# cunningham-lab/cyclic-gps

Hardware: AMD Instinct MI355X
Metric: block-tridiag solve+log-det (mahal_and_det) algorithmic GB/s vs HBM roofline, N=2^20 d=4 on one GPU, N=2^24 d=4 time-axis sharded on several; solves/s alongside (higher is better)
Workload: dtype f64; 1 GPU; BASELINE config 2: mahal_and_det on ONE SPD block-tridiagonal system, N=1048576 block rows (1048576 per GPU), d=4, conditioned bidiagonal-factor generator seed 1234; rows_total=1048576, rows_per_gpu=1048576, d=4, algorithmic_bytes=301989776, parallelism=single GPU, algo=tile-fused

## Files before the change

__graft_entry__.py:

```python
import os
import subprocess
import sys

ROOT = os.path.dirname(os.path.abspath(__file__))
PKG = os.path.join(ROOT, "cyclic-gps_amd")
CSRC = os.path.join(PKG, "csrc")
LIB = os.path.join(PKG, "lib", "libcgps.so")
HIPCC = os.environ.get("HIPCC", "/opt/rocm/bin/hipcc")


def _stale(target, sources):
    if not os.path.exists(target):
        return True
    t = os.path.getmtime(target)
    return any(os.path.getmtime(s) > t for s in sources)


UNITS = ("cgps_core", "cgps_mahal", "cgps_decompose", "cgps_solve", "cgps_inverse", "cgps_leg", "cgps_sample",
         "cgps_leg_obs")
FLAGS = ["--offload-arch=gfx950", "-O3", "-std=c++17", "-fPIC", "-Wno-unused-value"]
FLAGS += os.environ.get("CGPS_CXXFLAGS", "").split()


def _compile_unit(args):
    src, obj = args
    cmd = [HIPCC] + FLAGS + ["-c", src, "-o", obj]
    print("[build]", " ".join(cmd), flush=True)
    subprocess.check_call(cmd, cwd=ROOT)
    return obj


def build_oracle():
    if ROOT not in sys.path:
        sys.path.insert(0, ROOT)
    from oracle import cr_oracle


def build(force=False):
    from concurrent.futures import ThreadPoolExecutor
    hdrs = [os.path.join(CSRC, f) for f in sorted(os.listdir(CSRC)) if f.endswith(".h")]
    hdrs.append(os.path.join(ROOT, "include", "cgps.h"))
    objdir = os.path.join(PKG, "lib", "obj")
    os.makedirs(objdir, exist_ok=True)
    jobs, objs = [], []
    stamp = os.path.join(objdir, ".flags")
    flag_key = " ".join(FLAGS)
    flags_changed = (open(stamp).read() if os.path.exists(stamp) else None) != flag_key
    for u in UNITS:
        src, obj = os.path.join(CSRC, u + ".hip"), os.path.join(objdir, u + ".o")
        objs.append(obj)
        if force or flags_changed or _stale(obj, [src] + hdrs):
            jobs.append((src, obj))
    if jobs:
        with ThreadPoolExecutor(max_workers=min(len(jobs), os.cpu_count() or 4)) as ex:
            list(ex.map(_compile_unit, jobs))
        with open(stamp, "w") as fh:
            fh.write(flag_key)
    if jobs or _stale(LIB, objs):
        cmd = [HIPCC, "--offload-arch=gfx950", "-shared", "-fPIC", "-o", LIB] + objs
        print("[build]", " ".join(cmd), flush=True)
        subprocess.check_call(cmd, cwd=ROOT)
    for p in (ROOT, PKG):
        if p not in sys.path:
            sys.path.insert(0, p)
    from cyclic_gps import _hip
    assert _hip.lib().cgps_version() >= 100
    import cyclic_gps.cyclic_reduction
    build_oracle()
    print("[build] libcgps.so version", _hip.lib().cgps_version(), "exports", len(_hip.exported_symbols()), "symbols")


def smoke():
    import torch
    for p in (ROOT, PKG, os.path.join(ROOT, "tests")):
        if p not in sys.path:
            sys.path.insert(0, p)
    import cyclic_gps.cyclic_reduction as cr
    from oracle import cr_oracle
    import _util
    assert torch.cuda.is_available(), "smoke() needs a GPU"
# ... 21 lines not shown
```

cyclic-gps_amd/csrc/cgps_tile.h:

```cpp
#pragma once
#include <cstdlib>
#include <map>
#include <mutex>
#include <utility>
#include <type_traits>

#include "cgps_level.h"
#include "cgps_plan.h"
#include "cgps_leg.h"

namespace cgps {
#include "cgps_tile_leg.h"

template <typename T, int D>
struct LdsTile {
  static constexpr int DD = D * D;
  static constexpr int VN = Vec16<T>::N;
  static constexpr int G = (DD % VN == 0) ? DD / VN : 0;
  static constexpr bool SWZ = G >= 2 && (G & (G - 1)) == 0;
  T* R;
  T* Oc;
  T* y;
  static __device__ __forceinline__ int key(int row) { return (row ^ (row >> 3) ^ (row >> 6) ^ (row >> 9)) & (G - 1); }

// ... 162 lines not shown
    }                                                                                            \
  } while (0)
#else
#define CGPS_STAMP(slot) do { } while (0)
#endif

#include "cgps_tile_mfma.h"
#include "cgps_tile_quad.h"

#ifndef CGPS_MFMA_WIDE
#define CGPS_MFMA_WIDE 1
#endif
#ifndef CGPS_TILE_QUAD
#define CGPS_TILE_QUAD 1
#endif
#ifndef CGPS_QUAD4_MIN_ELIM
#define CGPS_QUAD4_MIN_ELIM(nthr) ((nthr) / 16)
#endif
#ifndef CGPS_TILE_QUAD4
#define CGPS_TILE_QUAD4 1
#endif
template <typename T, int D, int NTHR, int MW = CGPS_MFMA_WIDE>
__device__ __forceinline__ int tile_cr(LdsTile<T, D>& t, int n_real, PivotLog& pl, double& mah, bool& fail,
                                       long long* stamps = nullptr) {
  int stamp_pass = 0;
  (void)stamp_pass;
  static_assert(NTHR % 256 == 0, "tile_cr wants a multiple of four waves");
  using LT = LdsTile<T, D>;
  constexpr int NGRP = NTHR / 256;
  constexpr int DH = (D + 1) / 2;
  const int lane = threadIdx.x & 63, wave = threadIdx.x >> 6;
  const int role = wave & 3, grp = wave >> 2;
  const int K = n_real - 1;
  int levels = 0;
  int opaque_tid = threadIdx.x;
  if constexpr (D == 8 || D == 4) asm volatile("" : "+v"(opaque_tid));
#pragma unroll 1
  for (int s = 1; (s - 1) < K; s <<= 1, ++levels) {
    const int M = (K + 1) / s, h = s >> 1;
    const int n_elim = (M + 1) / 2;
    if constexpr (D == 8 && CGPS_TILE_QUAD) {
      tile_cr_level_quad<T, D, NTHR>(t, opaque_tid, K, M, s, pl, mah, fail);
      continue;
    }
    if constexpr (D == 4 && CGPS_TILE_QUAD4) {
      if (!std::is_same<T, double>::value || n_elim > CGPS_QUAD4_MIN_ELIM(NTHR)) {
        tile_cr_level_quad<T, D, NTHR>(t, opaque_tid, K, M, s, pl, mah, fail);
        continue;
      }
    }
    if constexpr (std::is_same<T, double>::value && D == 4) {
      constexpr int PER = NTHR / 16;
      if (n_elim <= PER) { tile_cr_level_mfma<NTHR, 1>(t, K, M, s, pl, mah, fail); continue; }
      if constexpr (MW >= 2) {
        if (n_elim <= 2 * PER) { tile_cr_level_mfma<NTHR, 2>(t, K, M, s, pl, mah, fail); continue; }
      }
      if constexpr (MW >= 4) {
        if (n_elim <= 4 * PER) { tile_cr_level_mfma<NTHR, 4>(t, K, M, s, pl, mah, fail); continue; }
      }
    }
#pragma unroll 1
// ... 135 lines not shown
  }
}

constexpr int FOLD_SLOTS = 1024;
constexpr int FOLD_SLOT_LDS_STAGES = 1 << 16;
#ifndef CGPS_FOLD_GROUP
#define CGPS_FOLD_GROUP 16
#endif
constexpr int FOLD_GROUP = CGPS_FOLD_GROUP;
constexpr int FOLD_MAX_GROUPS = 64;
static __device__ unsigned int g_fold_counter[FOLD_SLOTS][1 + FOLD_MAX_GROUPS];

template <typename T, int D> constexpr int record_rcmax() { return (D == 8 || (sizeof(T) == 8 && D == 6)) ? 1 : 4; }

template <typename T, int D>
struct RecordLayout {
  static constexpr int DD = D * D;
  static constexpr int STRIDE = record_stride(D);
  static constexpr int RS = 0, CS = DD, DRA = 2 * DD, YS = 3 * DD, DYA = 3 * DD + D;
};


template <typename T, int D>
__device__ __forceinline__ void collect_left_updates(LdsTile<T, D>& t, int levels, T (&dRa)[D][D], T (&dya)[D]) {
  for (int l = 0; l < levels; ++l) {
    const int slot = (1 << l) - 1;
    T P[D][D], p[D];
    LdsTile<T, D>::load_blk(t.R, slot, P);
    load_vec<T, D>(t.y + slot * D, p);
#pragma unroll
    for (int i = 0; i < D; ++i) {
      dya[i] -= p[i];
#pragma unroll
      for (int j = 0; j <= i; ++j) dRa[i][j] -= P[i][j];
    }
  }
}

constexpr int FAIL_LATE = 0x40000000;
__device__ __forceinline__ int fail_code(bool early, bool any, int64_t row) {
  const int r = (int)(row < (int64_t)(FAIL_LATE - 2) ? row : (int64_t)(FAIL_LATE - 2)) + 1;
  return early ? r : (any ? (r | FAIL_LATE) : 0);
}
template <int NT>
__device__ __forceinline__ void write_partial(double mah, double logp, int failrow_plus1, double* __restrict__ partial,
                                              double* red, int* sfail) {
  if (failrow_plus1) atomicMin(sfail, failrow_plus1);
  block_sum2<NT>(mah, logp, red);
// ... 47 lines not shown
  if constexpr (NT > 64) {
    if (lane == 63 && w < NT / 64 - 1) {
      const T* p = xch + w * (DD + D);
#pragma unroll
      for (int i = 0; i < D; ++i) {
#pragma unroll
        for (int j2 = 0; j2 <= i; ++j2) nR[i][j2] = p[i * D + j2];
        ny[i] = p[DD + i];
      }
    }
  }
  if (tid < n_real - 1) {
#pragma unroll
    for (int i = 0; i < D; ++i) {
#pragma unroll
      for (int j2 = 0; j2 <= i; ++j2) Rc[i][j2] += nR[i][j2];
      yc[i] += ny[i];
    }
  }
}

template <typename T, int D, int NT>
__device__ __forceinline__ void reduce_staged_tile_and_emit(LdsTile<T, D>& t, int n_real, T* xch, T* __restrict__ rec_out,
                                                            PivotLog& pl, double& mah, bool& fail);
template <typename T, int D, int NT>
__device__ __forceinline__ void reduce_tile_and_emit(LdsTile<T, D>& t, T (&Rc)[D][D], T (&yc)[D], T (&Cc)[D][D],
                                                     T (&dRa)[D][D], T (&dya)[D], int n_real, T* xch,
                                                     T* __restrict__ rec_out, PivotLog& pl, double& mah, bool& fail) {
  using RL = RecordLayout<T, D>;
  const int tid = threadIdx.x;
  absorb_right_neighbour_update<T, D, NT>(Rc, yc, dRa, dya, xch, n_real);
  if (tid < n_real) {
    mirror_lower<T, D>(Rc);
    LdsTile<T, D>::store_blk(t.R, tid, Rc);
    store_vec<T, D>(t.y + tid * D, yc);
    LdsTile<T, D>::store_blk(t.Oc, tid, Cc);
  }
  if (tid == 0) {
#pragma unroll
    for (int i = 0; i < D; ++i) {
#pragma unroll
      for (int j = 0; j <= i; ++j) xch[i * D + j] = dRa[i][j];
      xch[D * D + i] = dya[i];
    }
  }
  reduce_staged_tile_and_emit<T, D, NT>(t, n_real, xch, rec_out, pl, mah, fail);
}

template <typename T, int D, int NT>
__device__ __forceinline__ void reduce_staged_tile_and_emit(LdsTile<T, D>& t, int n_real, T* xch, T* __restrict__ rec_out,
                                                            PivotLog& pl, double& mah, bool& fail) {
  using RL = RecordLayout<T, D>;
  const int tid = threadIdx.x;
  __syncthreads();
  CGPS_KSTAMP(8);
  const int levels = tile_cr<T, D, NT>(t, n_real, pl, mah, fail);
  CGPS_KSTAMP(9);
  if (rec_out != nullptr && tid < D * D) {
    using LT = LdsTile<T, D>;
    constexpr int VN = LT::VN;
    const int i = tid / D, j = tid % D;
    auto elem = [&](const T* base, int slot) {
      const int idx = i * D + j;
      const T* p = base + (size_t)slot * D * D;
      return LT::SWZ ? p[((idx / VN) ^ LT::key(slot)) * VN + (idx % VN)] : p[idx];
    };
    T dra = (i >= j) ? xch[i * D + j] : xch[j * D + i];
    T dyv = xch[D * D + i];
    for (int l = 0; l < levels; ++l) {
      const int slot = (1 << l) - 1;
      dra -= elem(t.R, slot);
      dyv -= t.y[slot * D + i];
    }
    T* r = rec_out;
    store_wt(r + RL::RS + tid, elem(t.R, n_real - 1));
    store_wt(r + RL::CS + tid, elem(t.Oc, 0));
    store_wt(r + RL::DRA + tid, dra);
    if (j == 0) {
      store_wt(r + RL::YS + i, t.y[(n_real - 1) * D + i]);
      store_wt(r + RL::DYA + i, dyv);
    }
  }
}

template <typename T, int D, int NTILE, int NT>
struct StageSmem {
  static constexpr int DD = D * D;
  LdsTile<T, D> t;
  double* red;
  T* xch;
  int* sfail;
  __device__ __forceinline__ StageSmem(char* smem) {
// ... 5 lines not shown
  }
};


template <typename T, int D> constexpr int stage1_row_group() {
  if (sizeof(T) == 8 && (D == 3 || D == 5)) return 2;
  return 1;
}
template <typename T, int D> constexpr int stage1_min_waves() {
  return ((sizeof(T) == 8 && D <= 4) || (sizeof(T) == 4 && D <= 5)) ? 2 : 1;
}
struct FoldArgs {
  int slot;
  void* group_records;
  double* out2;
  int* info;
  void* shard_record;
  double* shard_partial;
  int rows_per_lane;
  int pair_slot;
  size_t pair_ws_stride;
  const unsigned char* obs_pattern;
  int obs_entries;
};
#include "cgps_tile_rec.h"
template <typename T, int D, int NTILE, int NT, bool FINAL, bool INL = false>
__device__ __forceinline__ void record_reduce_body(char* smem, unsigned tile_index, const T* __restrict__ rin, int64_t n,
                                                   int rc, T* __restrict__ rout, double* __restrict__ partial_out,
                                                   const double* __restrict__ partial_in, int64_t n_partial,
                                                   double* __restrict__ out2, int* __restrict__ info,
                                                   int64_t rows_per_record, int64_t N, int64_t rstride, int64_t pstride);
template <typename T, int D, int NW, bool ONE_PER_CU>
__device__ __forceinline__ void fold_record_stages(char* smem, int* last_flag, T* __restrict__ rec, double* __restrict__ partial,
                                                   const FoldArgs& fold, int64_t rows_per_tile, int64_t N) {
  const int tid = threadIdx.x;
    constexpr bool COH = ONE_PER_CU && (D * D) % Vec16<T>::N == 0;
    using RL = RecordLayout<T, D>;
    const unsigned grp = blockIdx.x / FOLD_GROUP, ngrp = (gridDim.x + FOLD_GROUP - 1) / FOLD_GROUP;
    const unsigned gsize = (grp + 1 < ngrp) ? (unsigned)FOLD_GROUP : gridDim.x - grp * FOLD_GROUP;
    const int slot = fold.slot & (FOLD_SLOT_LDS_STAGES - 1);
    if constexpr (std::is_same<T, double>::value && D == 4 && FOLD_GROUP == fold_reg::MAX_RECORDS) {
      if (gridDim.x <= FOLD_GROUP * fold_reg::MAX_RECORDS && !(fold.slot & FOLD_SLOT_LDS_STAGES)) {
        if (tid >= 64) return;
        int lane = tid;
        asm volatile("" : "+v"(lane));
        auto arrive1 = [&](unsigned int* ctr, unsigned expected) {
          asm volatile("s_waitcnt vmcnt(0)" ::: "memory");
          int last = 0;
// ... 220 lines not shown
        leg_add_weighted_basis<T, D>(Oleft, reinterpret_cast<const T*>(fold.obs_pattern), fold.obs_entries, rn, cR);
        leg_row<T, D>(Rg, Og, (const T*)nullptr, yg, rn, N, cR, cB, Rn, On, yn, fail);
      } else
        leg_row<T, D>(Rg, Og, Oleft, yg, rn, N, cR, cB, Rn, On, yn, fail);
      eliminate_forward<T, D>(Rc, yc, Cc, dRa, dya, On, Rn, yn, pl, mah, fail);
      continue;
    }
    load_block<T, D>(Rg + rn * DD, Rn);
    load_block<T, D>(Og + (rn - 1) * DD, On);
    if (yfull) {
      if (((j + 1) & (YR - 1)) == 0) stage_y_line(rn);
      load_vec<T, D>(ylds + ((j + 1) & (YR - 1)) * D, yn);
    } else {
      load_vec<T, D>(yg + rn * D, yn);
    }
    eliminate_forward<T, D>(Rc, yc, Cc, dRa, dya, On, Rn, yn, pl, mah, fail);
  }
  }

  CGPS_KSTAMP(1);
  const bool fail_stream = fail;
  int64_t nreal64 = (N + C - 1) / C - lane0;
  const int n_real = nreal64 > NT ? NT : (int)nreal64;
  reduce_tile_and_emit<T, D, NW>(sm.t, Rc, yc, Cc, dRa, dya, n_real, sm.xch, rec + (size_t)blockIdx.x * RecordLayout<T, D>::STRIDE,
                                 pl, mah, fail);
  CGPS_KSTAMP(2);
  int64_t frow = r0 < N ? r0 : N - 1;
  write_partial<NW>(mah, pl.value(), fail_code(fail_stream, fail, frow), partial + PARTIAL_STRIDE * (size_t)blockIdx.x, sm.red, sm.sfail);
  CGPS_KSTAMP(3);
  if constexpr (FOLD)
    fold_record_stages<T, D, NW, (NW == 2 * NT)>(smem, sm.sfail + 1, rec, partial, fold, (int64_t)C * NT, N);
}

template <typename T, int D>
__device__ __forceinline__ void load_record_row(const T* __restrict__ rin, int64_t rstride, int64_t w, int64_t n,
                                                bool add_next, T (&R)[D][D], T (&y)[D], T (&Cs)[D][D]) {
  using RL = RecordLayout<T, D>;
  if (w < n) {
    const T* r = rin + (size_t)w * rstride;
    load_block<T, D>(r + RL::RS, R);
    load_vec<T, D>(r + RL::YS, y);
    load_block<T, D>(r + RL::CS, Cs);
    if (add_next && w + 1 < n) {
      const T* q = rin + (size_t)(w + 1) * rstride;
      T nR[D][D], ny[D];
      load_block<T, D>(q + RL::DRA, nR);
      load_vec<T, D>(q + RL::DYA, ny);
#pragma unroll
// ... 291 lines not shown
    (void)hipFuncSetAttribute(reinterpret_cast<const void*>(&chunk_reduce_kernel<T, D, 8, Cfg::NT1, Cfg::NT1, true>),
                              hipFuncAttributeMaxDynamicSharedMemorySize, lds1);
    (void)hipFuncSetAttribute(reinterpret_cast<const void*>(&chunk_reduce_kernel<T, D, 4, Cfg::NT1>),
                              hipFuncAttributeMaxDynamicSharedMemorySize, lds1);
    (void)hipFuncSetAttribute(reinterpret_cast<const void*>(&chunk_reduce_kernel<T, D, 4, Cfg::NT1, Cfg::NT1, true>),
                              hipFuncAttributeMaxDynamicSharedMemorySize, lds1);
    (void)hipFuncSetAttribute(reinterpret_cast<const void*>(&chunk_reduce_kernel<T, D, 1, Cfg::NT1>),
                              hipFuncAttributeMaxDynamicSharedMemorySize, lds1);
    (void)hipFuncSetAttribute(reinterpret_cast<const void*>(&chunk_reduce_kernel<T, D, 1, Cfg::NT1, Cfg::NT1, true>),
                              hipFuncAttributeMaxDynamicSharedMemorySize, lds1);
  }
  (void)hipFuncSetAttribute(reinterpret_cast<const void*>(&record_reduce_kernel<T, D, Cfg::NTILE3, Cfg::NT3, false>),
                            hipFuncAttributeMaxDynamicSharedMemorySize, lds3);
  (void)hipFuncSetAttribute(reinterpret_cast<const void*>(&record_reduce_kernel<T, D, Cfg::NTILE3, Cfg::NT3, true>),
                            hipFuncAttributeMaxDynamicSharedMemorySize, lds3);
  });
}

inline bool fold_reg_enabled() {
  static const bool on = [] { const char* e = getenv("CGPS_FOLD_REG"); return !(e && e[0] == '0'); }();
  return on;
}

static int fold_slot_for(const void* ws) {
  static std::mutex mu;
  static std::map<std::pair<int, const void*>, int> slots;
  static std::pair<int, const void*> owner[FOLD_SLOTS];
  static unsigned long long last_use[FOLD_SLOTS];
  static unsigned long long tick = 0;
  int dev = 0;
  (void)hipGetDevice(&dev);
  const std::pair<int, const void*> key{dev, ws};
  std::lock_guard<std::mutex> lock(mu);
  auto it = slots.find(key);
  int s;
  if (it != slots.end()) {
    s = it->second;
  } else if ((int)slots.size() < FOLD_SLOTS) {
    s = (int)slots.size();
    slots.emplace(key, s);
    owner[s] = key;
  } else {
    s = 0;
    for (int k = 1; k < FOLD_SLOTS; ++k)
      if (last_use[k] < last_use[s]) s = k;
    slots.erase(owner[s]);
// ... 58 lines not shown
  const int64_t tiles = (N + rows_per_tile - 1) / rows_per_tile;
  double* partial = cgps_host::at<double>(ws, w.partial);
  T* recA = cgps_host::at<T>(ws, w.recA);
  T* recB = cgps_host::at<T>(ws, w.recB);
  const size_t lds1 = stage_lds_bytes<T, D>(Cfg::NG1, Cfg::NT1), lds3 = stage_lds_bytes<T, D>(Cfg::NTILE3, Cfg::NT3);
  tile_set_attributes<T, D>();
  if (ev_start) (void)hipEventRecord(ev_start, st);
  if constexpr (Cfg::LPR > 1) {
    const int slot = (tiles > 1 && tiles <= (int64_t)FOLD_GROUP * FOLD_MAX_GROUPS && fold_final_enabled()) ? fold_slot_for(ws) : -1;
    if (slot >= 0) {
      const FoldArgs fa{slot, recB, out2, info, shard_record, shard_partial};
      hipLaunchKernelGGL((chunk_reduce_ml_kernel<T, D, Cfg::C, Cfg::NT1, Cfg::LPR, true>), dim3((unsigned)tiles),
                         dim3(Cfg::NT1), lds1, st, Rs, Os, x, N, Oleft, recA, partial, fa);
      if (ev_stop) (void)hipEventRecord(ev_stop, st);
      return 0;
    }
    hipLaunchKernelGGL((chunk_reduce_ml_kernel<T, D, Cfg::C, Cfg::NT1, Cfg::LPR>), dim3((unsigned)tiles), dim3(Cfg::NT1),
                       lds1, st, Rs, Os, x, N, Oleft, recA, partial, FoldArgs{});
  }
  else if constexpr (Cfg::ALWAYS_WIDE) {
    const int slot = (tiles > 1 && tiles <= (int64_t)FOLD_GROUP * FOLD_MAX_GROUPS && fold_final_enabled()) ? fold_slot_for(ws) : -1;
    const size_t ldsw = stage_lds_bytes<T, D>(Cfg::NG1, 2 * Cfg::NT1);
    if (slot >= 0 && clong > 0) {
      const FoldArgs fa{slot, recB, out2, info, shard_record, shard_partial, clong};
      hipLaunchKernelGGL((chunk_reduce_kernel<T, D, 0, Cfg::NT1, 2 * Cfg::NT1, true>), dim3((unsigned)tiles),
                         dim3(2 * Cfg::NT1), ldsw, st, Rs, Os, x, N, Oleft, recA, partial, fa);
      if (ev_stop) (void)hipEventRecord(ev_stop, st);
      return 0;
    }
    if (slot >= 0) {
      const FoldArgs fa{slot, recB, out2, info, shard_record, shard_partial};
      hipLaunchKernelGGL((chunk_reduce_kernel<T, D, Cfg::C, Cfg::NT1, 2 * Cfg::NT1, true>), dim3((unsigned)tiles),
                         dim3(2 * Cfg::NT1), ldsw, st, Rs, Os, x, N, Oleft, recA, partial, fa);
      if (ev_stop) (void)hipEventRecord(ev_stop, st);
      return 0;
    }
    hipLaunchKernelGGL((chunk_reduce_kernel<T, D, Cfg::C, Cfg::NT1, 2 * Cfg::NT1>), dim3((unsigned)tiles),
                       dim3(2 * Cfg::NT1), ldsw, st, Rs, Os, x, N, Oleft, recA, partial, FoldArgs{});
  } else if (clong > 0) {
    const int slot = fold_slot_for(ws);
    const FoldArgs fa{slot, recB, out2, info, shard_record, shard_partial, clong};
    bool wide = false;
    if constexpr (stage1_min_waves<T, D>() == 2) {
      if (!long_chunk_narrow()) {
        wide = true;
        const size_t ldsw = stage_lds_bytes<T, D>(Cfg::NG1, 2 * Cfg::NT1);
        hipLaunchKernelGGL((chunk_reduce_kernel<T, D, 0, Cfg::NT1, 2 * Cfg::NT1, true>), dim3((unsigned)tiles),
                           dim3(2 * Cfg::NT1), ldsw, st, Rs, Os, x, N, Oleft, recA, partial, fa);
      }
    }
    if (!wide)
      hipLaunchKernelGGL((chunk_reduce_kernel<T, D, 0, Cfg::NT1, Cfg::NT1, true>), dim3((unsigned)tiles), dim3(Cfg::NT1),
                         lds1, st, Rs, Os, x, N, Oleft, recA, partial, fa);
    if (ev_stop) (void)hipEventRecord(ev_stop, st);
    return 0;
  } else if (csel != Cfg::C) {
    const int slot = (fold_final_enabled() && !(shard_record != nullptr && tiles == 1)) ? fold_slot_for(ws) : -1;
    const FoldArgs fa{slot, recB, out2, info, shard_record, shard_partial};
    auto launch = [&](auto cs) {
      constexpr int CS = decltype(cs)::value;
      if (slot >= 0)
        hipLaunchKernelGGL((chunk_reduce_kernel<T, D, CS, Cfg::NT1, Cfg::NT1, true>), dim3((unsigned)tiles), dim3(Cfg::NT1),
                           lds1, st, Rs, Os, x, N, Oleft, recA, partial, fa);
      else
        hipLaunchKernelGGL((chunk_reduce_kernel<T, D, CS, Cfg::NT1>), dim3((unsigned)tiles), dim3(Cfg::NT1), lds1, st,
                           Rs, Os, x, N, Oleft, recA, partial, FoldArgs{});
    };
    if (csel == 1) launch(std::integral_constant<int, 1>{});
    else if (csel == 4) launch(std::integral_constant<int, 4>{});
    else launch(std::integral_constant<int, 8>{});
    if (slot >= 0) {
      if (ev_stop) (void)hipEventRecord(ev_stop, st);
      return 0;
    }
  }
  else {
    const int slot = (tiles > 1 && tiles <= (int64_t)FOLD_GROUP * FOLD_MAX_GROUPS && fold_final_enabled()) ? fold_slot_for(ws) : -1;
    const FoldArgs fa{slot, recB, out2, info, shard_record, shard_partial};
    bool wide = false;
    if constexpr (stage1_min_waves<T, D>() == 2) {
      if (tiles <= STAGE1_SMALL_TILES) {
        wide = true;
        const size_t ldsw = stage_lds_bytes<T, D>(Cfg::NG1, 2 * Cfg::NT1);
        if (slot >= 0)
          hipLaunchKernelGGL((chunk_reduce_kernel<T, D, Cfg::C, Cfg::NT1, 2 * Cfg::NT1, true>), dim3((unsigned)tiles),
                             dim3(2 * Cfg::NT1), ldsw, st, Rs, Os, x, N, Oleft, recA, partial, fa);
        else
          hipLaunchKernelGGL((chunk_reduce_kernel<T, D, Cfg::C, Cfg::NT1, 2 * Cfg::NT1>), dim3((unsigned)tiles),
                             dim3(2 * Cfg::NT1), ldsw, st, Rs, Os, x, N, Oleft, recA, partial, FoldArgs{});
      }
    }
    if (!wide) {
      if (slot >= 0)
        hipLaunchKernelGGL((chunk_reduce_kernel<T, D, Cfg::C, Cfg::NT1, Cfg::NT1, true>), dim3((unsigned)tiles), dim3(Cfg::NT1),
                           lds1, st, Rs, Os, x, N, Oleft, recA, partial, fa);
      else
        hipLaunchKernelGGL((chunk_reduce_kernel<T, D, Cfg::C, Cfg::NT1>), dim3((unsigned)tiles), dim3(Cfg::NT1), lds1, st,
                           Rs, Os, x, N, Oleft, recA, partial, FoldArgs{});
    }
    if (slot >= 0) {
      if (ev_stop) (void)hipEventRecord(ev_stop, st);
      return 0;
    }
  }
  if (ev_stop) (void)hipEventRecord(ev_stop, st);
  int64_t n = tiles, npart = tiles, rows_per_record = rows_per_tile;
  T *rin = recA, *rout = recB;
  while (shard_record ? n > 1 : n > (int64_t)Cfg::NTILE3 * Cfg::RCMAX) {
    int rc = (int)((n + Cfg::NTILE3 - 1) / Cfg::NTILE3);
    if (rc > Cfg::RCMAX) rc = Cfg::RCMAX;
    const int64_t per = (int64_t)Cfg::NTILE3 * rc;
    const int64_t g = (n + per - 1) / per;
    const bool shard_last = shard_record && g == 1;
    if (shard_last) rout = shard_record;
    hipLaunchKernelGGL((record_reduce_kernel<T, D, Cfg::NTILE3, Cfg::NT3, false>), dim3((unsigned)g), dim3(Cfg::NT3),
                       lds3, st, (const T*)rin, n, rc, rout, shard_last ? shard_partial : partial + PARTIAL_STRIDE * npart,
                       shard_last ? (const double*)partial : (const double*)nullptr, shard_last ? npart : (int64_t)0,
                       (double*)nullptr, (int*)nullptr, rows_per_record, N, (int64_t)RL::STRIDE,
                       (int64_t)PARTIAL_STRIDE);
    if (shard_last) return 0;
    npart += g;
// ... 76 lines not shown
```

cyclic-gps_amd/csrc/dev_bench.hip:

```cpp
#include <hip/hip_runtime.h>

#include <cmath>
#include <cstdio>
#include <cstdlib>
#include <vector>

#define CGPS_FIN_STAMPS 1
#ifndef DEVB_D
#define DEVB_D 4
#endif
#ifndef DEVB_T
#define DEVB_T double
#endif
#include "cgps_tile.h"

using namespace cgps;

template <typename T, int D>
__device__ __forceinline__ void set_identity(T (&A)[D][D]) {
#pragma unroll
  for (int i = 0; i < D; ++i)
#pragma unroll
    for (int j = 0; j < D; ++j) A[i][j] = (i == j) ? T(1) : T(0);
}
// ... 175 lines not shown
  double* sums;
  CK(hipMalloc(&ticks, grid * sizeof(long long)));
  CK(hipMalloc(&sums, 2 * grid * sizeof(double)));
  const int reps = 50;
  printf("tile_cr NTHR=%d MW=%d grid=%d :", NTHR, MW, grid);
  double prev = 0;
  for (int n_real : {2, 4, 8, 16, 32, 64, 128, 256}) {
    hipLaunchKernelGGL((tilecr_bench_kernel<NTHR, MW>), dim3(grid), dim3(NTHR), lds, st, n_real, reps, ticks, sums);
    CK(hipStreamSynchronize(st));
    std::vector<long long> h(grid);
    std::vector<double> hs(2 * grid);
    CK(hipMemcpy(h.data(), ticks, grid * sizeof(long long), hipMemcpyDeviceToHost));
    CK(hipMemcpy(hs.data(), sums, 2 * grid * sizeof(double), hipMemcpyDeviceToHost));
    double avg = 0;
    for (auto v : h) avg += (double)v;
    avg = avg / grid / reps * 10.0;
    printf("  n=%d: %.0f ns (+%.0f)", n_real, avg, avg - prev);
    if (n_real == 256) printf("  [check %.10g %.10g]", hs[0], hs[1]);
    prev = avg;
  }
  printf("\n");
  CK(hipFree(ticks));
  CK(hipFree(sums));
}

template <bool REG, bool FINAL>
__global__ __launch_bounds__(512) void record_stage_bench_kernel(const double* rec, int n, int reps, double* rout, double* pout,
                                                                 const double* pin, int n_partial, double* out2, int* info,
                                                                 long long* ticks) {
  extern __shared__ __attribute__((aligned(16))) char smem[];
  using RL = RecordLayout<double, 4>;
  long long acc = 0;
  for (int rep = 0; rep < reps; ++rep) {
    __syncthreads();
    const long long t0 = wall_clock64();
    if constexpr (REG) {
      if (threadIdx.x < 64)
        record_stage_reg<true>((int)threadIdx.x, FINAL, rec, n, rout, pout, FINAL ? pin : nullptr, FINAL ? n_partial : 0, out2, info,
                                      0, 4096, (int64_t)n * 4096);
    } else {
      record_reduce_body<double, 4, (FINAL ? FOLD_MAX_GROUPS : FOLD_GROUP), 512, FINAL, true>(smem, 0u, rec, (int64_t)n, 1, rout, pout, FINAL ? pin : nullptr,
                                                                  FINAL ? (int64_t)n_partial : 0, out2, info, 4096,
                                                                  (int64_t)n * 4096, (int64_t)RL::STRIDE, (int64_t)PARTIAL_STRIDE);
    }
    asm volatile("s_waitcnt vmcnt(0)" ::: "memory");
    const long long t1 = wall_clock64();
// ... 138 lines not shown
        long long st[16];
        CK(hipMemcpyFromSymbol(st, HIP_SYMBOL(g_fin_stamps), sizeof(st)));
        double o[2];
        CK(hipMemcpy(o, out2, 16, hipMemcpyDeviceToHost));
        if (it >= 28) {
          static long long ks[512][12];
          CK(hipMemcpyFromSymbol(ks, HIP_SYMBOL(g_k_stamps), sizeof(ks)));
          long long t0 = ks[0][0];
          for (int b = 0; b < 256; ++b) t0 = ks[b][0] < t0 ? ks[b][0] : t0;
          static int xcc[512];
          CK(hipMemcpyFromSymbol(xcc, HIP_SYMBOL(g_k_xcc), sizeof(xcc)));
          double sx[8] = {0}, mx[8] = {0};
          int cx[8] = {0};
          for (int b = 0; b < 256; ++b) {
            const int x = xcc[b] & 7;
            const double d = (ks[b][1] - t0) * 0.01;
            sx[x] += d; cx[x]++; mx[x] = d > mx[x] ? d : mx[x];
          }
          printf("   stream end per XCD (avg/max us):");
          for (int x = 0; x < 8; ++x) printf(" [%d: n=%d %.1f/%.1f]", x, cx[x], cx[x] ? sx[x] / cx[x] : 0.0, mx[x]);
          printf("\n   stream end by block index (us):");
          for (int b = 0; b < 256; b += 17) printf(" b%d:%.1f", b, (ks[b][1] - t0) * 0.01);
          printf("\n");
          const char* names[10] = {"start", "streamed", "tile reduced+emitted", "partial written", "arrived(group)",
                                   "group reduced", "arrived(top)", "final done", "rows staged in LDS", "tile_cr done"};
          for (int k = 0; k < 10; ++k) {
            long long lo = 1LL << 62, hi = 0;
            int cnt = 0;
            for (int b = 0; b < 256; ++b) {
              if (ks[b][k] < t0) continue;
              lo = ks[b][k] < lo ? ks[b][k] : lo;
              hi = ks[b][k] > hi ? ks[b][k] : hi;
              ++cnt;
            }
            if (cnt) printf("   %-22s first %.2f us  last %.2f us  (%d workgroups)\n", names[k], (lo - t0) * 0.01, (hi - t0) * 0.01, cnt);
          }
        }
        if (it >= 27)
          printf("mode %s rc %d: op %.1f us | final: loads %.2f  lds-stores %.2f  reduce %.2f  last-row %.2f  sums+write %.2f  total %.2f us  [%.10g %.10g]\n",
                 mode == 0 ? "two launches" : "folded", rc, ms * 1e3, (st[1] - st[0]) * 0.01, (st[2] - st[1]) * 0.01,
                 (st[3] - st[2]) * 0.01, (st[4] - st[3]) * 0.01, (st[5] - st[4]) * 0.01, (st[5] - st[0]) * 0.01, o[0], o[1]);
      }
      break;
    }
    return 0;
  }
  if (argc > 2 && atoi(argv[2]) == 3) {
    hipStream_t s3;
    CK(hipStreamCreate(&s3));
    run_record_stages(s3);
    return 0;
  }
  if (argc > 2 && atoi(argv[2]) == 1) {
    hipStream_t s2;
    CK(hipStreamCreate(&s2));
    for (int grid : {1, 256}) {
      run_tilecr<256, 1>(grid, s2);
      run_tilecr<256, 2>(grid, s2);
      run_tilecr<256, 4>(grid, s2);
      run_tilecr<512, 1>(grid, s2);
      run_tilecr<512, 2>(grid, s2);
      run_tilecr<512, 4>(grid, s2);
    }
    return 0;
  }
  hipStream_t st;
  CK(hipStreamCreate(&st));
  T *R, *O, *y;
  double* out;
  CK(hipMalloc(&R, N * D * D * sizeof(T)));
  CK(hipMalloc(&O, N * D * D * sizeof(T)));
  CK(hipMalloc(&y, N * D * sizeof(T)));
  CK(hipMalloc(&out, 4096));
  hipLaunchKernelGGL((gen_kernel<T, D>), dim3((unsigned)((N + 255) / 256)), dim3(256), 0, st, R, O, y, N);
  CK(hipStreamSynchronize(st));
// ... 23 lines not shown
```

Before: 4543 GB/s.

## Run first cyclic-reduction levels in registers via DPP before LDS staging

```diff
diff --git a/__graft_entry__.py b/__graft_entry__.py
--- a/__graft_entry__.py
+++ b/__graft_entry__.py
@@ -22,12 +22,62 @@
 FLAGS += os.environ.get("CGPS_CXXFLAGS", "").split()
 
 
+RESOURCE_UNIT = "cgps_mahal"
+
+
+def _resource_report(obj):
+    return obj[:-2] + ".resources.txt"
+
+
 def _compile_unit(args):
     src, obj = args
     cmd = [HIPCC] + FLAGS + ["-c", src, "-o", obj]
+    if os.path.basename(src) == RESOURCE_UNIT + ".hip":
+        cmd.insert(len(cmd) - 4, "-Rpass-analysis=kernel-resource-usage")
+        print("[build]", " ".join(cmd), flush=True)
+        r = subprocess.run(cmd, cwd=ROOT, stderr=subprocess.PIPE, text=True)
+        with open(_resource_report(obj), "w") as fh:
+            fh.write(r.stderr)
+        rest = [l for l in r.stderr.splitlines() if "-Rpass-analysis=kernel-resource-usage" not in l]
+        if rest:
+            print("\n".join(rest), file=sys.stderr, flush=True)
+        if r.returncode != 0:
+            raise subprocess.CalledProcessError(r.returncode, cmd)
+        return obj
     print("[build]", " ".join(cmd), flush=True)
     subprocess.check_call(cmd, cwd=ROOT)
     return obj
+
+
+def kernel_resources(report):
+    import re
+    out, cur = {}, None
+    for line in open(report, errors="replace"):
+        m = re.search(r"Function Name: (\S+)", line)
+        if m:
+            cur = out.setdefault(m.group(1), {})
+            continue
+        m = re.search(r":  +([A-Za-z ]+?)(?: \[[^\]]*\])?: (\d+) \[-Rpass", line)
+        if m and cur is not None:
+            cur.setdefault(m.group(1), int(m.group(2)))
+    return out
+
+
+def check_kernel_resources(report):
+    res = kernel_resources(report)
+    mine = {k: v for k, v in res.items() if "chunk_reduce_kernelIdLi4E" in k and k.split("EEEv")[0].endswith("ELi0")}
+    if not mine:
+        raise RuntimeError("no kernel-resource-usage remarks for chunk_reduce_kernel<double, 4, ..., SRC = 0> in " + report)
+    bad = ["%s: %d bytes of scratch per lane" % (k, v["ScratchSize"]) for k, v in mine.items() if v.get("ScratchSize", 0) != 0]
+    head = [v for k, v in mine.items() if "chunk_reduce_kernelIdLi4ELi16ELi256ELi512ELb1ELi0E" in k]
+    if len(head) != 1:
+        bad.append("headline kernel chunk_reduce_kernel<double, 4, 16, 256, 512, true, 0>: %d reports" % len(head))
+    elif head[0].get("VGPRs", 0) + head[0].get("AGPRs", 0) > 256:
+        bad.append("headline kernel: %d VGPRs + %d AGPRs" % (head[0]["VGPRs"], head[0]["AGPRs"]))
+    if bad:
+        raise RuntimeError("kernel resource check failed:\n  " + "\n  ".join(bad))
+    print("[build] resource check: %d chunk_reduce_kernel<double, 4, .., SRC = 0> instantiations without scratch; headline %d VGPRs"
+          % (len(mine), head[0]["VGPRs"]))
 
 
 def build_oracle():
@@ -49,13 +99,14 @@
     for u in UNITS:
         src, obj = os.path.join(CSRC, u + ".hip"), os.path.join(objdir, u + ".o")
         objs.append(obj)
-        if force or flags_changed or _stale(obj, [src] + hdrs):
+        if force or flags_changed or _stale(obj, [src] + hdrs) or (u == RESOURCE_UNIT and not os.path.exists(_resource_report(obj))):
             jobs.append((src, obj))
     if jobs:
         with ThreadPoolExecutor(max_workers=min(len(jobs), os.cpu_count() or 4)) as ex:
             list(ex.map(_compile_unit, jobs))
         with open(stamp, "w") as fh:
             fh.write(flag_key)
+    check_kernel_resources(_resource_report(os.path.join(objdir, RESOURCE_UNIT + ".o")))
     if jobs or _stale(LIB, objs):
         cmd = [HIPCC, "--offload-arch=gfx950", "-shared", "-fPIC", "-o", LIB] + objs
         print("[build]", " ".join(cmd), flush=True)
diff --git a/cyclic-gps_amd/csrc/cgps_tile.h b/cyclic-gps_amd/csrc/cgps_tile.h
--- a/cyclic-gps_amd/csrc/cgps_tile.h
+++ b/cyclic-gps_amd/csrc/cgps_tile.h
@@ -208,7 +208,7 @@
 #endif
 template <typename T, int D, int NTHR, int MW = CGPS_MFMA_WIDE>
 __device__ __forceinline__ int tile_cr(LdsTile<T, D>& t, int n_real, PivotLog& pl, double& mah, bool& fail,
-                                       long long* stamps = nullptr) {
+                                       long long* stamps = nullptr, int first = 0) {
   int stamp_pass = 0;
   (void)stamp_pass;
   static_assert(NTHR % 256 == 0, "tile_cr wants a multiple of four waves");
@@ -222,7 +222,7 @@
   int opaque_tid = threadIdx.x;
   if constexpr (D == 8 || D == 4) asm volatile("" : "+v"(opaque_tid));
 #pragma unroll 1
-  for (int s = 1; (s - 1) < K; s <<= 1, ++levels) {
+  for (int s = 1 << first; (s - 1) < K; s <<= 1, ++levels) {
     const int M = (K + 1) / s, h = s >> 1;
     const int n_elim = (M + 1) / 2;
     if constexpr (D == 8 && CGPS_TILE_QUAD) {
@@ -404,8 +404,8 @@
 
 
 template <typename T, int D>
-__device__ __forceinline__ void collect_left_updates(LdsTile<T, D>& t, int levels, T (&dRa)[D][D], T (&dya)[D]) {
-  for (int l = 0; l < levels; ++l) {
+__device__ __forceinline__ void collect_left_updates(LdsTile<T, D>& t, int levels, T (&dRa)[D][D], T (&dya)[D], int first = 0) {
+  for (int l = first; l < first + levels; ++l) {
     const int slot = (1 << l) - 1;
     T P[D][D], p[D];
     LdsTile<T, D>::load_blk(t.R, slot, P);
@@ -499,12 +499,20 @@
 
 template <typename T, int D, int NT>
 __device__ __forceinline__ void reduce_staged_tile_and_emit(LdsTile<T, D>& t, int n_real, T* xch, T* __restrict__ rec_out,
-                                                            PivotLog& pl, double& mah, bool& fail);
+                                                            PivotLog& pl, double& mah, bool& fail, int first = 0);
+template <typename T, int D, int NT>
+__device__ __forceinline__ void stage_kept_rows(LdsTile<T, D>& t, T (&Rc)[D][D], T (&yc)[D], T (&Cc)[D][D],
+                                                T (&dRa)[D][D], T (&dya)[D], int n_real, T* xch);
 template <typename T, int D, int NT>
 __device__ __forceinline__ void reduce_tile_and_emit(LdsTile<T, D>& t, T (&Rc)[D][D], T (&yc)[D], T (&Cc)[D][D],
                                                      T (&dRa)[D][D], T (&dya)[D], int n_real, T* xch,
                                                      T* __restrict__ rec_out, PivotLog& pl, double& mah, bool& fail) {
-  using RL = RecordLayout<T, D>;
+  stage_kept_rows<T, D, NT>(t, Rc, yc, Cc, dRa, dya, n_real, xch);
+  reduce_staged_tile_and_emit<T, D, NT>(t, n_real, xch, rec_out, pl, mah, fail);
+}
+template <typename T, int D, int NT>
+__device__ __forceinline__ void stage_kept_rows(LdsTile<T, D>& t, T (&Rc)[D][D], T (&yc)[D], T (&Cc)[D][D],
+                                                T (&dRa)[D][D], T (&dya)[D], int n_real, T* xch) {
   const int tid = threadIdx.x;
   absorb_right_neighbour_update<T, D, NT>(Rc, yc, dRa, dya, xch, n_real);
   if (tid < n_real) {
@@ -521,17 +529,16 @@
       xch[D * D + i] = dya[i];
     }
   }
-  reduce_staged_tile_and_emit<T, D, NT>(t, n_real, xch, rec_out, pl, mah, fail);
 }
 
 template <typename T, int D, int NT>
 __device__ __forceinline__ void reduce_staged_tile_and_emit(LdsTile<T, D>& t, int n_real, T* xch, T* __restrict__ rec_out,
-                                                            PivotLog& pl, double& mah, bool& fail) {
+                                                            PivotLog& pl, double& mah, bool& fail, int first) {
   using RL = RecordLayout<T, D>;
   const int tid = threadIdx.x;
   __syncthreads();
   CGPS_KSTAMP(8);
-  const int levels = tile_cr<T, D, NT>(t, n_real, pl, mah, fail);
+  const int levels = tile_cr<T, D, NT>(t, n_real, pl, mah, fail, nullptr, first);
   CGPS_KSTAMP(9);
   if (rec_out != nullptr && tid < D * D) {
     using LT = LdsTile<T, D>;
@@ -544,7 +551,7 @@
     };
     T dra = (i >= j) ? xch[i * D + j] : xch[j * D + i];
     T dyv = xch[D * D + i];
-    for (int l = 0; l < levels; ++l) {
+    for (int l = first; l < first + levels; ++l) {
       const int slot = (1 << l) - 1;
       dra -= elem(t.R, slot);
       dyv -= t.y[slot * D + i];
@@ -596,8 +603,10 @@
   size_t pair_ws_stride;
   const unsigned char* obs_pattern;
   int obs_entries;
+  int wave_levels;
 };
 #include "cgps_tile_rec.h"
+#include "cgps_tile_wave.h"
 template <typename T, int D, int NTILE, int NT, bool FINAL, bool INL = false>
 __device__ __forceinline__ void record_reduce_body(char* smem, unsigned tile_index, const T* __restrict__ rin, int64_t n,
                                                    int rc, T* __restrict__ rout, double* __restrict__ partial_out,
@@ -864,8 +873,23 @@
   const bool fail_stream = fail;
   int64_t nreal64 = (N + C - 1) / C - lane0;
   const int n_real = nreal64 > NT ? NT : (int)nreal64;
-  reduce_tile_and_emit<T, D, NW>(sm.t, Rc, yc, Cc, dRa, dya, n_real, sm.xch, rec + (size_t)blockIdx.x * RecordLayout<T, D>::STRIDE,
-                                 pl, mah, fail);
+  if constexpr (SRC == 0 && std::is_same<T, double>::value && D == 4 && CGPS_WAVE_LEVELS > 0) {
+    int first = 0;
+    if (fold.wave_levels != 0 && n_real == NT) {
+      int otid = tid;
+      asm volatile("" : "+v"(otid));
+      wave_levels_and_hand_over<CGPS_WAVE_LEVELS, NT>(sm.t, otid, Rc, yc, Cc, dRa, dya, sm.xch, pl, mah, fail);
+      CGPS_KSTAMP(10);
+      first = CGPS_WAVE_LEVELS;
+    } else {
+      stage_kept_rows<T, D, NW>(sm.t, Rc, yc, Cc, dRa, dya, n_real, sm.xch);
+    }
+    reduce_staged_tile_and_emit<T, D, NW>(sm.t, n_real, sm.xch, rec + (size_t)blockIdx.x * RecordLayout<T, D>::STRIDE, pl, mah,
+                                          fail, first);
+  } else {
+    reduce_tile_and_emit<T, D, NW>(sm.t, Rc, yc, Cc, dRa, dya, n_real, sm.xch, rec + (size_t)blockIdx.x * RecordLayout<T, D>::STRIDE,
+                                   pl, mah, fail);
+  }
   CGPS_KSTAMP(2);
   int64_t frow = r0 < N ? r0 : N - 1;
   write_partial<NW>(mah, pl.value(), fail_code(fail_stream, fail, frow), partial + PARTIAL_STRIDE * (size_t)blockIdx.x, sm.red, sm.sfail);
@@ -1203,6 +1227,15 @@
   return on;
 }
 
+inline bool wave_levels_enabled() {
+  static const bool on = [] { const char* e = getenv("CGPS_WAVE_LEVELS"); return !(e && e[0] == '0'); }();
+  return on;
+}
+inline FoldArgs with_wave_levels(FoldArgs fa) {
+  fa.wave_levels = wave_levels_enabled() ? CGPS_WAVE_LEVELS : 0;
+  return fa;
+}
+
 static int fold_slot_for(const void* ws) {
   static std::mutex mu;
   static std::map<std::pair<int, const void*>, int> slots;
@@ -1307,24 +1340,24 @@
     const int slot = (tiles > 1 && tiles <= (int64_t)FOLD_GROUP * FOLD_MAX_GROUPS && fold_final_enabled()) ? fold_slot_for(ws) : -1;
     const size_t ldsw = stage_lds_bytes<T, D>(Cfg::NG1, 2 * Cfg::NT1);
     if (slot >= 0 && clong > 0) {
-      const FoldArgs fa{slot, recB, out2, info, shard_record, shard_partial, clong};
+      const FoldArgs fa = with_wave_levels(FoldArgs{slot, recB, out2, info, shard_record, shard_partial, clong});
       hipLaunchKernelGGL((chunk_reduce_kernel<T, D, 0, Cfg::NT1, 2 * Cfg::NT1, true>), dim3((unsigned)tiles),
                          dim3(2 * Cfg::NT1), ldsw, st, Rs, Os, x, N, Oleft, recA, partial, fa);
       if (ev_stop) (void)hipEventRecord(ev_stop, st);
       return 0;
     }
     if (slot >= 0) {
-      const FoldArgs fa{slot, recB, out2, info, shard_record, shard_partial};
+      const FoldArgs fa = with_wave_levels(FoldArgs{slot, recB, out2, info, shard_record, shard_partial});
       hipLaunchKernelGGL((chunk_reduce_kernel<T, D, Cfg::C, Cfg::NT1, 2 * Cfg::NT1, true>), dim3((unsigned)tiles),
                          dim3(2 * Cfg::NT1), ldsw, st, Rs, Os, x, N, Oleft, recA, partial, fa);
       if (ev_stop) (void)hipEventRecord(ev_stop, st);
       return 0;
     }
     hipLaunchKernelGGL((chunk_reduce_kernel<T, D, Cfg::C, Cfg::NT1, 2 * Cfg::NT1>), dim3((unsigned)tiles),
-                       dim3(2 * Cfg::NT1), ldsw, st, Rs, Os, x, N, Oleft, recA, partial, FoldArgs{});
+                       dim3(2 * Cfg::NT1), ldsw, st, Rs, Os, x, N, Oleft, recA, partial, with_wave_levels(FoldArgs{}));
   } else if (clong > 0) {
     const int slot = fold_slot_for(ws);
-    const FoldArgs fa{slot, recB, out2, info, shard_record, shard_partial, clong};
+    const FoldArgs fa = with_wave_levels(FoldArgs{slot, recB, out2, info, shard_record, shard_partial, clong});
     bool wide = false;
     if constexpr (stage1_min_waves<T, D>() == 2) {
       if (!long_chunk_narrow()) {
@@ -1341,7 +1374,7 @@
     return 0;
   } else if (csel != Cfg::C) {
     const int slot = (fold_final_enabled() && !(shard_record != nullptr && tiles == 1)) ? fold_slot_for(ws) : -1;
-    const FoldArgs fa{slot, recB, out2, info, shard_record, shard_partial};
+    const FoldArgs fa = with_wave_levels(FoldArgs{slot, recB, out2, info, shard_record, shard_partial});
     auto launch = [&](auto cs) {
       constexpr int CS = decltype(cs)::value;
       if (slot >= 0)
@@ -1349,7 +1382,7 @@
                            lds1, st, Rs, Os, x, N, Oleft, recA, partial, fa);
       else
         hipLaunchKernelGGL((chunk_reduce_kernel<T, D, CS, Cfg::NT1>), dim3((unsigned)tiles), dim3(Cfg::NT1), lds1, st,
-                           Rs, Os, x, N, Oleft, recA, partial, FoldArgs{});
+                           Rs, Os, x, N, Oleft, recA, partial, with_wave_levels(FoldArgs{}));
     };
     if (csel == 1) launch(std::integral_constant<int, 1>{});
     else if (csel == 4) launch(std::integral_constant<int, 4>{});
@@ -1361,7 +1394,7 @@
   }
   else {
     const int slot = (tiles > 1 && tiles <= (int64_t)FOLD_GROUP * FOLD_MAX_GROUPS && fold_final_enabled()) ? fold_slot_for(ws) : -1;
-    const FoldArgs fa{slot, recB, out2, info, shard_record, shard_partial};
+    const FoldArgs fa = with_wave_levels(FoldArgs{slot, recB, out2, info, shard_record, shard_partial});
     bool wide = false;
     if constexpr (stage1_min_waves<T, D>() == 2) {
       if (tiles <= STAGE1_SMALL_TILES) {
@@ -1372,7 +1405,7 @@
                              dim3(2 * Cfg::NT1), ldsw, st, Rs, Os, x, N, Oleft, recA, partial, fa);
         else
           hipLaunchKernelGGL((chunk_reduce_kernel<T, D, Cfg::C, Cfg::NT1, 2 * Cfg::NT1>), dim3((unsigned)tiles),
-                             dim3(2 * Cfg::NT1), ldsw, st, Rs, Os, x, N, Oleft, recA, partial, FoldArgs{});
+                             dim3(2 * Cfg::NT1), ldsw, st, Rs, Os, x, N, Oleft, recA, partial, with_wave_levels(FoldArgs{}));
       }
     }
     if (!wide) {
@@ -1381,7 +1414,7 @@
                            lds1, st, Rs, Os, x, N, Oleft, recA, partial, fa);
       else
         hipLaunchKernelGGL((chunk_reduce_kernel<T, D, Cfg::C, Cfg::NT1>), dim3((unsigned)tiles), dim3(Cfg::NT1), lds1, st,
-                           Rs, Os, x, N, Oleft, recA, partial, FoldArgs{});
+                           Rs, Os, x, N, Oleft, recA, partial, with_wave_levels(FoldArgs{}));
     }
     if (slot >= 0) {
       if (ev_stop) (void)hipEventRecord(ev_stop, st);
diff --git a/cyclic-gps_amd/csrc/cgps_tile_wave.h b/cyclic-gps_amd/csrc/cgps_tile_wave.h
--- /dev/null
+++ b/cyclic-gps_amd/csrc/cgps_tile_wave.h
@@ -0,0 +1,107 @@
+#pragma once
+
+#ifndef CGPS_WAVE_LEVELS
+#define CGPS_WAVE_LEVELS 2
+#endif
+
+namespace wave_levels {
+constexpr int MAX_LEVELS = 4;
+constexpr bool pulls(int lane, int l) { return (lane & ((2 << l) - 1)) == (2 << l) - 1; }
+constexpr int pull_source(int lane, int l) { return lane - (1 << l); }
+constexpr int surviving_slot(int m, int L) { return (m + 1) * (1 << L) - 1; }
+constexpr bool survives(int lane, int L) { return (lane & ((1 << L) - 1)) == (1 << L) - 1; }
+constexpr int parking_slot(int o, int L) { return o < (2 << (L - 1)) ? -1 : o - (1 << (L - 1)); }
+constexpr int coupling_slot(int o, int L) { return o - (1 << L) + 1; }
+}
+
+#ifdef __HIPCC__
+template <int S>
+__device__ __forceinline__ double row_shr_f64(double v) {
+  static_assert(S >= 1 && S <= 15, "row_shr:1..15");
+  const int lo = __builtin_amdgcn_mov_dpp(__double2loint(v), 0x110 + S, 0xf, 0xf, false);
+  const int hi = __builtin_amdgcn_mov_dpp(__double2hiint(v), 0x110 + S, 0xf, 0xf, false);
+  return __hiloint2double(hi, lo);
+}
+
+template <int LV>
+__device__ __forceinline__ void wave_level(int lane, double (&Rc)[4][4], double (&yc)[4], double (&Cc)[4][4],
+                                           double (&dRa)[4][4], double (&dya)[4], PivotLog& pl, double& mah, bool& fail) {
+  constexpr int D = 4, S = 1 << LV;
+  static_assert(wave_levels::pull_source(15, LV) >= 0, "the source is in the same 16-lane row");
+  double eR[D][D], ey[D], eC[D][D], edR[D][D], edy[D];
+#pragma unroll
+  for (int i = 0; i < D; ++i) {
+#pragma unroll
+    for (int j = 0; j < D; ++j) {
+      eC[i][j] = row_shr_f64<S>(Cc[i][j]);
+      if (j <= i) {
+        eR[i][j] = row_shr_f64<S>(Rc[i][j]);
+        edR[i][j] = row_shr_f64<S>(dRa[i][j]);
+      } else {
+        eR[i][j] = 0.0;
+        edR[i][j] = 0.0;
+      }
+    }
+    ey[i] = row_shr_f64<S>(yc[i]);
+    edy[i] = row_shr_f64<S>(dya[i]);
+  }
+  if (wave_levels::pulls(lane, LV)) {
+#pragma unroll
+    for (int i = 0; i < D; ++i) {
+      ey[i] += dya[i];
+#pragma unroll
+      for (int j = 0; j <= i; ++j) eR[i][j] += dRa[i][j];
+    }
+    eliminate_forward<double, D>(eR, ey, eC, edR, edy, Cc, Rc, yc, pl, mah, fail);
+#pragma unroll
+    for (int i = 0; i < D; ++i) {
+      dya[i] = edy[i];
+#pragma unroll
+      for (int j = 0; j < D; ++j) {
+        Cc[i][j] = eC[i][j];
+        if (j <= i) dRa[i][j] = edR[i][j];
+      }
+    }
+  }
+}
+
+template <int L, int NT>
+__device__ __forceinline__ void wave_levels_and_hand_over(LdsTile<double, 4>& t, int tid, double (&Rc)[4][4], double (&yc)[4],
+                                                          double (&Cc)[4][4], double (&dRa)[4][4], double (&dya)[4],
+                                                          double* xch, PivotLog& pl, double& mah, bool& fail) {
+  static_assert(L >= 1 && L <= wave_levels::MAX_LEVELS && NT % 64 == 0, "row shifts of 1, 2, 4 and 8 lanes");
+  constexpr int D = 4;
+  using LT = LdsTile<double, D>;
+  if (tid >= NT) return;
+  wave_level<0>(tid, Rc, yc, Cc, dRa, dya, pl, mah, fail);
+  if constexpr (L >= 2) wave_level<1>(tid, Rc, yc, Cc, dRa, dya, pl, mah, fail);
+  if constexpr (L >= 3) wave_level<2>(tid, Rc, yc, Cc, dRa, dya, pl, mah, fail);
+  if constexpr (L >= 4) wave_level<3>(tid, Rc, yc, Cc, dRa, dya, pl, mah, fail);
+  if (wave_levels::survives(tid, L)) {
+    mirror_lower<double, D>(Rc);
+    LT::store_blk(t.R, tid, Rc);
+    store_vec<double, D>(t.y + tid * D, yc);
+    LT::store_blk(t.Oc, wave_levels::coupling_slot(tid, L), Cc);
+    if (tid == wave_levels::surviving_slot(0, L)) {
+#pragma unroll
+      for (int i = 0; i < D; ++i) {
+#pragma unroll
+        for (int j = 0; j <= i; ++j) xch[i * D + j] = dRa[i][j];
+        xch[D * D + i] = dya[i];
+      }
+    } else {
+      const int park = tid - (1 << (L - 1));
+      double P[D][D], p[D];
+#pragma unroll
+      for (int i = 0; i < D; ++i) {
+        p[i] = -dya[i];
+#pragma unroll
+        for (int j = 0; j <= i; ++j) P[i][j] = -dRa[i][j];
+      }
+      mirror_lower<double, D>(P);
+      LT::store_blk(t.R, park, P);
+      store_vec<double, D>(t.y + park * D, p);
+    }
+  }
+}
+#endif
diff --git a/cyclic-gps_amd/csrc/dev_bench.hip b/cyclic-gps_amd/csrc/dev_bench.hip
--- a/cyclic-gps_amd/csrc/dev_bench.hip
+++ b/cyclic-gps_amd/csrc/dev_bench.hip
@@ -221,6 +221,142 @@
   printf("\n");
   CK(hipFree(ticks));
   CK(hipFree(sums));
+}
+
+template <int L, int NTHR>
+__global__ __launch_bounds__(NTHR) void wave_levels_bench_kernel(int reps, long long* ticks, double* diff, double* sums, double* snap) {
+  constexpr int D = 4, NT = 256, S = 1 << L;
+  using LT = LdsTile<double, D>;
+  extern __shared__ __attribute__((aligned(16))) char smem[];
+  StageSmem<double, D, NT, NTHR> sm(smem);
+  const int tid = threadIdx.x;
+  long long acc[2] = {0, 0};
+  double mahs[2] = {0.0, 0.0}, logs[2] = {0.0, 0.0};
+  double worst = 0.0;
+  for (int rep = 0; rep < reps; ++rep) {
+#pragma unroll
+    for (int form = 0; form < 2; ++form) {
+      double Rc[D][D], yc[D], Cc[D][D], dRa[D][D], dya[D];
+      unsigned h = (unsigned)((tid + 977 * rep) * 2654435761u) ^ 0x9e3779b9u;
+      auto rnd = [&]() { h = h * 1664525u + 1013904223u; return (double)((h >> 8) & 0xffff) / 65536.0 - 0.5; };
+      for (int a = 0; a < D; ++a) {
+        for (int b = 0; b <= a; ++b) {
+          const double v = (a == b) ? 2.5 + 0.2 * rnd() : 0.1 * rnd(), u = (a == b) ? -0.2 - 0.1 * rnd() : 0.02 * rnd();
+          Rc[a][b] = v; Rc[b][a] = v; dRa[a][b] = u; dRa[b][a] = u;
+        }
+        for (int b = 0; b < D; ++b) Cc[a][b] = 0.3 * rnd();
+        yc[a] = rnd();
+        dya[a] = 0.1 * rnd();
+      }
+      if (tid >= NT) { set_zero<double, D>(Rc); set_zero<double, D>(yc); set_zero<double, D>(Cc); set_zero<double, D>(dRa); set_zero<double, D>(dya); }
+      PivotLog pl;
+      double mah = 0.0;
+      bool fail = false;
+      __syncthreads();
+      const long long t0 = wall_clock64();
+      if (form == 0) {
+        stage_kept_rows<double, D, NTHR>(sm.t, Rc, yc, Cc, dRa, dya, NT, sm.xch);
+        __syncthreads();
+        for (int s = 1; s < S; s <<= 1) tile_cr_level_quad<double, D, NTHR>(sm.t, tid, NT - 1, NT / s, s, pl, mah, fail);
+      } else {
+        wave_levels_and_hand_over<L, NT>(sm.t, tid, Rc, yc, Cc, dRa, dya, sm.xch, pl, mah, fail);
+        __syncthreads();
+      }
+      const long long t1 = wall_clock64();
+      acc[form] += t1 - t0;
+      mahs[form] += mah;
+      logs[form] += pl.value();
+      if (rep == reps - 1 && tid < NT && wave_levels::survives(tid, L)) {
+        double A[D][D], B[D][D], P[D][D], a[D], p[D];
+        LT::load_blk(sm.t.R, tid, A);
+        LT::load_blk(sm.t.Oc, wave_levels::coupling_slot(tid, L), B);
+        load_vec<double, D>(sm.t.y + tid * D, a);
+        if (tid + (S >> 1) < NT - 1) {
+          double Q[D][D], q[D];
+          LT::load_blk(sm.t.R, tid + (S >> 1), Q);
+          load_vec<double, D>(sm.t.y + (tid + (S >> 1)) * D, q);
+          for (int i = 0; i < D; ++i) {
+            a[i] -= q[i];
+            for (int j = 0; j < D; ++j) A[i][j] -= Q[i][j];
+          }
+        }
+        if (wave_levels::parking_slot(tid, L) >= 0) {
+          set_zero<double, D>(P);
+          set_zero<double, D>(p);
+        } else {
+          for (int i = 0; i < D; ++i) {
+            p[i] = sm.xch[D * D + i];
+            for (int j = 0; j < D; ++j) P[i][j] = (i >= j) ? sm.xch[i * D + j] : sm.xch[j * D + i];
+          }
+          if (form == 0)
+            for (int l = 0; l < L; ++l) {
+              double Q[D][D], q[D];
+              LT::load_blk(sm.t.R, (1 << l) - 1, Q);
+              load_vec<double, D>(sm.t.y + ((1 << l) - 1) * D, q);
+              for (int i = 0; i < D; ++i) {
+                p[i] -= q[i];
+                for (int j = 0; j < D; ++j) P[i][j] -= Q[i][j];
+              }
+            }
+        }
+        auto emit = [&](int idx, double v) {
+          double* q = snap + (size_t)tid * (3 * D * D + 2 * D) + idx;
+          if (form == 0) { *q = v; return; }
+          const double ref = fabs(*q), rel = fabs(v - *q) / (ref >= 1e-3 ? ref : 1e-3);
+          worst = (rel > worst || rel != rel) ? rel : worst;
+        };
+        for (int i = 0; i < D; ++i) {
+          emit(3 * D * D + i, a[i]);
+          emit(3 * D * D + D + i, p[i]);
+          for (int j = 0; j < D; ++j) {
+            emit(i * D + j, A[i][j]);
+            emit(D * D + i * D + j, B[i][j]);
+            emit(2 * D * D + i * D + j, P[i][j]);
+          }
+        }
+      }
+    }
+  }
+  for (int off = 32; off > 0; off >>= 1) {
+    const double o = __shfl_down(worst, off, 64);
+    worst = (o > worst || o != o) ? o : worst;
+  }
+  if ((tid & 63) == 0) diff[tid >> 6] = worst;
+  for (int form = 0; form < 2; ++form) {
+    __syncthreads();
+    double m = mahs[form], g = logs[form];
+    block_sum2<NTHR>(m, g, sm.red);
+    if (tid == 0) { ticks[form] = acc[form]; sums[2 * form] = m; sums[2 * form + 1] = g; }
+  }
+}
+
+template <int L, int NTHR>
+static void run_wave_levels(hipStream_t st) {
+  const size_t lds = stage_lds_bytes<double, 4>(256, NTHR);
+  CK(hipFuncSetAttribute(reinterpret_cast<const void*>(&wave_levels_bench_kernel<L, NTHR>), hipFuncAttributeMaxDynamicSharedMemorySize, (int)lds));
+  long long* ticks;
+  double *diff, *sums, *snap;
+  CK(hipMalloc(&snap, 256 * 56 * sizeof(double)));
+  CK(hipMalloc(&ticks, 2 * sizeof(long long)));
+  CK(hipMalloc(&diff, 8 * sizeof(double)));
+  CK(hipMalloc(&sums, 4 * sizeof(double)));
+  const int reps = 200;
+  for (int pass = 0; pass < 2; ++pass)
+    hipLaunchKernelGGL((wave_levels_bench_kernel<L, NTHR>), dim3(1), dim3(NTHR), lds, st, reps, ticks, diff, sums, snap);
+  CK(hipStreamSynchronize(st));
+  long long t[2];
+  double d[8], s[4], worst = 0.0;
+  CK(hipMemcpy(t, ticks, sizeof(t), hipMemcpyDeviceToHost));
+  CK(hipMemcpy(d, diff, sizeof(d), hipMemcpyDeviceToHost));
+  CK(hipMemcpy(s, sums, sizeof(s), hipMemcpyDeviceToHost));
+  for (int w = 0; w < NTHR / 64; ++w) worst = (d[w] > worst || d[w] != d[w]) ? d[w] : worst;
+  printf("first %d levels of a full 256-row tile, %d threads: staged + quad levels %6.0f ns | in registers + hand-over %6.0f ns"
+         "  (per level %.0f ns)  largest relative difference of the LDS state %.3g  [sums %.12g %.12g | %.12g %.12g]\n",
+         L, NTHR, (double)t[0] / reps * 10.0, (double)t[1] / reps * 10.0, (double)t[1] / reps * 10.0 / L, worst, s[0], s[1], s[2], s[3]);
+  CK(hipFree(ticks));
+  CK(hipFree(diff));
+  CK(hipFree(sums));
+  CK(hipFree(snap));
 }
 
 template <bool REG, bool FINAL>
@@ -405,9 +541,12 @@
           printf("\n   stream end by block index (us):");
           for (int b = 0; b < 256; b += 17) printf(" b%d:%.1f", b, (ks[b][1] - t0) * 0.01);
           printf("\n");
-          const char* names[10] = {"start", "streamed", "tile reduced+emitted", "partial written", "arrived(group)",
-                                   "group reduced", "arrived(top)", "final done", "rows staged in LDS", "tile_cr done"};
-          for (int k = 0; k < 10; ++k) {
+          const char* names[11] = {"start", "streamed", "tile reduced+emitted", "partial written", "arrived(group)",
+                                   "group reduced", "arrived(top)", "final done", "rows staged in LDS", "tile_cr done",
+                                   "in-register levels"};
+          const int order[11] = {0, 1, 10, 8, 9, 2, 3, 4, 5, 6, 7};
+          for (int ki = 0; ki < 11; ++ki) {
+            const int k = order[ki];
             long long lo = 1LL << 62, hi = 0;
             int cnt = 0;
             for (int b = 0; b < 256; ++b) {
@@ -434,6 +573,18 @@
     run_record_stages(s3);
     return 0;
   }
+  if (argc > 2 && atoi(argv[2]) == 4) {
+    hipStream_t s4;
+    CK(hipStreamCreate(&s4));
+    run_wave_levels<1, 512>(s4);
+    run_wave_levels<2, 512>(s4);
+    run_wave_levels<3, 512>(s4);
+    run_wave_levels<4, 512>(s4);
+    run_wave_levels<2, 256>(s4);
+    run_wave_levels<3, 256>(s4);
+    run_wave_levels<4, 256>(s4);
+    return 0;
+  }
   if (argc > 2 && atoi(argv[2]) == 1) {
     hipStream_t s2;
     CK(hipStreamCreate(&s2));
```

Result: faster. 4642 GB/s (median of 6 runs) (+2.2%).
